# haoheliu/voicefixer

Measured on AMD Instinct MI355X. Metric: seconds-of-44.1kHz-audio restored per wall-second, higher is better.
Workload: dtype f32

## Files before the change

include/vfx_hip.h:

```cpp
#ifndef VFX_HIP_H
#define VFX_HIP_H

#include <stddef.h>
#include <stdint.h>

#ifdef __cplusplus
extern "C" {
#endif

typedef void* vfx_stream_t;

#define VFX_OK 0
#define VFX_EINVAL (-1)
#define VFX_EALIGN (-2)
#define VFX_ERANGE (-3)
#define VFX_ENOTSUP (-4)

typedef struct {
    void* ptr;
    int64_t bstride, cstride, lstride;
    int64_t guard;
    const int32_t* rows;
} vfx_tensor;

// ... 25 lines not shown

#define VFX_PAD_ZERO 0
#define VFX_PAD_REFLECT 1

int vfx_version(void);

const char* vfx_build_id(void);

uint64_t vfx_launch_count(void);

int vfx_last_conv_tile(void);


int vfx_conv1d_f32(const vfx_tensor* x, const float* w_packed, const float* bias,
                   const vfx_tensor* res, const vfx_tensor* y, int B, int Cin, int Cout, int L,
                   int k, int dilation, int pad_mode, const vfx_act* act, vfx_stream_t stream);

int vfx_conv1d_f16(const vfx_tensor* x, const void* w_f16, const float* bias, const vfx_tensor* res,
                   const vfx_tensor* y, int B, int C, int L, int dilation, const vfx_act* act, int32_t* range_flag,
                   vfx_stream_t stream);

typedef struct {
    const float* w1_direct;
    const float* bias1;
    const float* w2_direct;
    const float* bias2;
    const float* w2_wino;
    const float* w2_wino4;
    const float* w1_wino4;
} vfx_resblock_w;
int vfx_resblock_f32(const vfx_tensor* x, const vfx_tensor* y, const vfx_resblock_w* w, int B, int C, int L,
                     int dilation, float slope, int post_act, float post_slope, vfx_stream_t stream);

int vfx_convtr1d_f32(const vfx_tensor* x, const float* w_packed, const float* bias,
                     const vfx_tensor* y, int B, int Cin, int Cout, int Lin, int stride,
                     const vfx_act* act, vfx_stream_t stream);

int vfx_conv2d_f32(const vfx_tensor* x, const float* w_packed, const float* bias,
                   const vfx_tensor* res, const vfx_tensor* y, int B, int Cin, int Cout, int H,
                   int pitch_log2, int ksize, const vfx_act* act, vfx_stream_t stream);

int vfx_convtr2d_3x3s2_f32(const vfx_tensor* x, const float* w_packed, const vfx_tensor* y,
                           int B, int Cin, int Cout, int h, int in_pitch_log2,
                           const vfx_act* act, vfx_stream_t stream);

int vfx_conv1d_cout1_f32(const vfx_tensor* x, const float* w, const float* bias,
                         const vfx_tensor* y, int B, int Cin, int L, int k, int pad_mode,
                         int post_act, int out_mask_log2, vfx_stream_t stream);

int vfx_avgpool2x2_f32(const vfx_tensor* x, const vfx_tensor* y, int B, int C, int H,
                       int pitch_log2, vfx_stream_t stream);


int vfx_frontend_init(const float* window, const float* twiddle, const int32_t* lo,
                      const int32_t* hi, const int32_t* off, const float* coef, int nnz);

int vfx_frontend_readback(int which, int32_t* lo, int32_t* hi, int32_t* off, float* coef, int coef_capacity,
                          int* nnz_out);

int vfx_stft_mel_f32(const float* wav, int64_t wav_stride, int B, int N, float* mel,
                     vfx_stream_t stream);

int vfx_stft_mel_rows_f32(const float* wav, int64_t wav_stride, int B, const int32_t* n_rows, int T, float* mel,
                          vfx_stream_t stream);

int vfx_frontend_init_oracle(const int32_t* lo, const int32_t* hi, const int32_t* off, const float* coef,
// ... 48 lines not shown
```

voicefixer_amd/_lib.py:

```python
import ctypes as C
import os
import subprocess

from ._dev import dev_env

_HERE = os.path.dirname(os.path.abspath(__file__))
LIB_PATH = dev_env("VFX_LIB", os.path.join(_HERE, "libvfx_hip.so"))
CSRC = os.path.join(_HERE, "csrc")


class VfxError(RuntimeError):
    pass


class vfx_tensor(C.Structure):
    _fields_ = [("ptr", C.c_void_p), ("bstride", C.c_int64), ("cstride", C.c_int64),
                ("lstride", C.c_int64), ("guard", C.c_int64), ("rows", C.c_void_p)]


class vfx_act(C.Structure):
    _fields_ = [("pre_act", C.c_int), ("pre_slope", C.c_float), ("pre_scale", C.c_void_p),
                ("pre_shift", C.c_void_p), ("post_act", C.c_int), ("post_slope", C.c_float),
                ("math", C.c_int), ("w_x3", C.c_void_p), ("w_direct", C.c_void_p), ("w_wino4", C.c_void_p)]


class vfx_resblock_w(C.Structure):
    _fields_ = [("w1_direct", C.c_void_p), ("bias1", C.c_void_p), ("w2_direct", C.c_void_p), ("bias2", C.c_void_p),
                ("w2_wino", C.c_void_p), ("w2_wino4", C.c_void_p), ("w1_wino4", C.c_void_p)]


PRE_NONE, PRE_LRELU, PRE_AFFINE_LRELU = 0, 1, 2
POST_NONE, POST_LRELU, POST_ELU, POST_TANH, POST_SIGMOID, POST_LRELU_SNAKE = 0, 1, 2, 3, 4, 5
PAD_ZERO, PAD_REFLECT = 0, 1
MATH_F32, MATH_BF16X3 = 0, 1
EINVAL, EALIGN, ERANGE, ENOTSUP = -1, -2, -3, -4

_T = C.POINTER(vfx_tensor)
_A = C.POINTER(vfx_act)
_P = C.c_void_p
_I = C.c_int

SIGNATURES = {
    "vfx_version": (_I, []),
    "vfx_build_id": (C.c_char_p, []),
    "vfx_launch_count": (C.c_uint64, []),
    "vfx_last_conv_tile": (_I, []),
    "vfx_conv1d_f32": (_I, [_T, _P, _P, _T, _T, _I, _I, _I, _I, _I, _I, _I, _A, _P]),
    "vfx_conv1d_f16": (_I, [_T, _P, _P, _T, _T, _I, _I, _I, _I, _A, _P, _P]),
    "vfx_resblock_f32": (_I, [_T, _T, C.POINTER(vfx_resblock_w), _I, _I, _I, _I, C.c_float, _I, C.c_float, _P]),
    "vfx_convtr1d_f32": (_I, [_T, _P, _P, _T, _I, _I, _I, _I, _I, _A, _P]),
    "vfx_conv2d_f32": (_I, [_T, _P, _P, _T, _T, _I, _I, _I, _I, _I, _I, _A, _P]),
    "vfx_convtr2d_3x3s2_f32": (_I, [_T, _P, _T, _I, _I, _I, _I, _I, _A, _P]),
    "vfx_conv1d_cout1_f32": (_I, [_T, _P, _P, _T, _I, _I, _I, _I, _I, _I, _I, _P]),
    "vfx_avgpool2x2_f32": (_I, [_T, _T, _I, _I, _I, _I, _P]),
    "vfx_frontend_init": (_I, [_P, _P, _P, _P, _P, _P, _I]),
    "vfx_frontend_readback": (_I, [_I, _P, _P, _P, _P, _I, C.POINTER(_I)]),
    "vfx_stft_mel_f32": (_I, [_P, C.c_int64, _I, _I, _P, _P]),
    "vfx_stft_mel_rows_f32": (_I, [_P, C.c_int64, _I, _P, _I, _P, _P]),
    "vfx_post_rows_f32": (_I, [_P, C.c_int64, _I, _P, _P, C.c_int64, _P, _I, _I, _P, _P]),
    "vfx_mel_to_cond_rows_f32": (_I, [_P, _T, _I, _I, _P, _I, _P]),
    "vfx_frontend_init_oracle": (_I, [_P, _P, _P, _P, _I]),
    "vfx_peak_f32": (_I, [_P, C.c_int64, _I, _I, _P, _P]),
    "vfx_stft_mel_oracle_f32": (_I, [_P, C.c_int64, _I, _I, _P, _P, _P]),
    "vfx_mel_to_cond_ex_f32": (_I, [_P, _T, _I, _I, _I, _P]),
    "vfx_hf_workspace_bytes": (C.c_size_t, [_I, _I]),
    "vfx_hf_cut_f32": (_I, [_P, C.c_int64, _I, _I, _P, C.c_int64, C.c_float, _P, C.c_size_t, _P, _P]),
    "vfx_tm_to_cm_f32": (_I, [_P, _P, _I, _I, _I, C.c_int64, C.c_int64, _P]),
    "vfx_unet_input_f32": (_I, [_P, _T, _T, _I, _I, _I, _I, _P]),
    "vfx_unet_output_f32": (_I, [_T, _T, _P, _T, _P, _P, _I, _I, _I, _P]),
    "vfx_gru_bidir_f32": (_I, [_P, _P, _P, _T, _I, _I, _P]),
    "vfx_gru_bidir2_f32": (_I, [_P, _P, _P, _T, _I, _I, _P, C.c_size_t, _P, _P]),
    "vfx_gru_layout": (None, [C.POINTER(_I), C.POINTER(_I), C.POINTER(_I)]),
    "vfx_mel_to_cond_f32": (_I, [_P, _T, _I, _I, _P]),
    "vfx_post_f32": (_I, [_P, C.c_int64, _I, _P, C.c_int64, _I, _I, _P, _P]),
}

_lib = None


def build(verbose=False):
    r = subprocess.run(["make", "-C", CSRC, "-j8"], capture_output=True, text=True)
    if verbose or r.returncode != 0:
# ... 28 lines not shown
```

voicefixer_amd/csrc/vfx_conv.hip:

```cpp
#include "vfx_common.h"
#include <cstdio>
#include <cstdlib>
#include <cstring>
#include <map>
#include <mutex>
#include <string>
#include <type_traits>
#include <vector>

#ifndef VFX_X3_ABL
#define VFX_X3_ABL 0
#endif
#ifndef VFX_ABL
#define VFX_ABL 0
#endif
#define VFX_MAXPH 8
#define VFX_MAXT 9

typedef float f32x16 __attribute__((ext_vector_type(16)));
typedef unsigned int u32x4 __attribute__((ext_vector_type(4)));

#if VFX_ABL & 8
__device__ unsigned long long g_dbg[10];
__device__ unsigned long long g_dbgx[6];
// ... 53 lines not shown
    int q_shift, q_mask, o_rs, o_cs;
    int pad_mode, pre_act, post_act;
    float pre_slope, post_slope;
    int in_mask, out_mask;
    int tile_lo, tile_hi;
    int tpw;
    int x_guard;
    int ksplit, cpp, ws_ls;
    float* ws;
    int bl_step;
    int nxv;
    int res_init;
    const void* w3;
    const ConvTables* tab3;
    int segw3;
    int xplane3;
    int buf3;
    int bl3;
    int xrow3, wrow3;
    const float* wd;
    int kcx;
    int ntiles_l, xcd_chunk;
    int nph_fold;
    int wg_d;
    const int* x_rows;
    int lq_extra;
    int stagger, stagger_wgs;
    int w_tap0, w_tapstep, w_slab0, w_slabstep, w_slab_ph, w_ooff0, w_ooff_ph, w_nseg, w_seg0, w_segstep;
    const float* wd2;
    const float* bias2;
    int yp;
    float mid_slope;
    int rb_nq1;
};

template <int KC>
struct StageCfg {
    static constexpr int MAXXV = 4;
    static constexpr int MAXWV = KC == 16 ? 6 : (KC == 8 ? 4 : 5);
};

template <int MAXXV, int MAXWV>
struct StageState {
    int x_l[MAXXV];
    int x_kc[MAXXV];
    int x_off[MAXXV];
    int w_off[MAXWV];
    float4 xv[MAXXV];
    float4 wv[MAXWV];
};

template <bool FAST, int MAXXV, int MAXWV>
__device__ __forceinline__ void stage_load(StageState<MAXXV, MAXWV>& st, const ConvArgs& a,
                                           const float* __restrict__ xb, int xcs, int c0, int lshift,
                                           __amdgpu_buffer_rsrc_t xrsrc, __amdgpu_buffer_rsrc_t wrsrc, int Lin_row) {
    if constexpr (FAST) {
        const int xso = (c0 * xcs + lshift) * 4, wso = c0 * a.Cout * 4;
#pragma unroll
        for (int j = 0; j < MAXXV; ++j) {
            const u32x4 r = __builtin_amdgcn_raw_buffer_load_b128(xrsrc, st.x_off[j], xso, 0);
            st.xv[j] = make_float4(__uint_as_float(r.x), __uint_as_float(r.y), __uint_as_float(r.z), __uint_as_float(r.w));
        }
#pragma unroll
        for (int j = 0; j < MAXWV; ++j) {
            const u32x4 r = __builtin_amdgcn_raw_buffer_load_b128(wrsrc, st.w_off[j], wso, 0);
            st.wv[j] = make_float4(__uint_as_float(r.x), __uint_as_float(r.y), __uint_as_float(r.z), __uint_as_float(r.w));
// ... 908 lines not shown
    a.xs_floats = xs;
    return VFX_OK;
}



static float* splitk_workspace(hipStream_t s, size_t bytes) {
    static std::mutex mu;
    static std::map<std::pair<int, hipStream_t>, std::pair<float*, size_t>> pool;
    int dev = 0;
    if (hipGetDevice(&dev) != hipSuccess) return nullptr;
    std::lock_guard<std::mutex> lock(mu);
    auto& e = pool[std::make_pair(dev, s)];
    if (e.second < bytes) {
        static std::vector<float*> retired;
        if (e.first) retired.push_back(e.first);
        e.first = nullptr;
        e.second = 0;
        const size_t want = bytes + bytes / 2;
        if (hipMalloc((void**)&e.first, want) != hipSuccess) { e.first = nullptr; return nullptr; }
        e.second = want;
    }
    return e.first;
}


#include "vfx_convw.inc"
#include "vfx_convwg.inc"
#include "vfx_convwg4p.inc"
#include "vfx_convwg4x.inc"
#include "vfx_convtw.inc"
#include "vfx_convwg2d.inc"
#include "vfx_resblk4.inc"
#include "vfx_convh.inc"

template <int BM, int BL, int WGM, int WGL, int NT, int MODE, int ROWS = 1>
static int launch_x3_one(const ConvArgs& a, dim3 grid, size_t lds, hipStream_t s) {
    static unsigned long long attr_set = 0;
    int attr_dev = 0;
    if (hipGetDevice(&attr_dev) != hipSuccess) attr_dev = 0;
    auto kern = conv_x3_kernel<BM, BL, WGM, WGL, NT, MODE, ROWS>;
    if (!((attr_set >> (attr_dev & 63)) & 1ull)) {
        hipError_t e = hipFuncSetAttribute(reinterpret_cast<const void*>(kern),
                                           hipFuncAttributeMaxDynamicSharedMemorySize, 160 * 1024);
        if (e != hipSuccess) return (int)e;
        attr_set |= 1ull << (attr_dev & 63);
    }
    hipLaunchKernelGGL(kern, grid, dim3(256), lds, s, a);
    VFX_LAUNCHED();
    return vfx_last_error();
}

template <int BM, int BL, int WGM, int WGL>
static int launch_x3_tile(const ConvArgs& a, int nt, int mode, int rows, dim3 grid, size_t lds, hipStream_t s) {
    if (rows == 3 && nt == 3) return launch_x3_one<BM, BL, WGM, WGL, 3, 0, 3>(a, grid, lds, s);
    if (rows == 3) return launch_x3_one<BM, BL, WGM, WGL, 1, 0, 3>(a, grid, lds, s);
#define VFX_X3(NT_)                                                                                  \
    if (nt == NT_)                                                                                   \
        return mode == 2   ? launch_x3_one<BM, BL, WGM, WGL, NT_, 2>(a, grid, lds, s)                \
               : mode == 1 ? launch_x3_one<BM, BL, WGM, WGL, NT_, 1>(a, grid, lds, s)                \
                           : launch_x3_one<BM, BL, WGM, WGL, NT_, 0>(a, grid, lds, s);
    VFX_X3(1)
    VFX_X3(2)
    VFX_X3(3)
#undef VFX_X3
    return VFX_ENOTSUP;
// ... 408 lines not shown
```

voicefixer_amd/csrc/vfx_resblk4.inc:

```
__global__ __launch_bounds__(256, 2) void resblk4_kernel(const ConvArgs a) {
    constexpr int C = 64, KC = 16, NSTEP = KC / 2, S = C / KC;
    constexpr int BQ = 64, CG = 256 / BQ, NSLOT = KC / CG;
    constexpr int PLANE = KC * BQ, BUF = 6 * PLANE;
    static_assert(NSTEP / NSLOT == 2, "two k-pair steps per staged element");
    extern __shared__ __attribute__((aligned(16))) float smem[];

    const int tid = threadIdx.x, lane = tid & 63;
    const int wave = __builtin_amdgcn_readfirstlane(tid >> 6);
    const int lo = lane & 31, hi = lane >> 5;
    const int wm = wave & 1, wq = wave >> 1;
    int bx = blockIdx.x;
    if (a.xcd_chunk > 0) {
        bx = (bx & 7) * a.xcd_chunk + (bx >> 3);
        if (bx >= a.ntiles_l) return;
    }
    const int b = blockIdx.z;
    const int d = a.wg_d;
    const float inv_d = 1.0f / (float)d;
    const int Lrow = a.x_rows ? __builtin_amdgcn_readfirstlane(a.x_rows[b]) : a.Lin;
    const int q0 = bx * a.bl_step;
    if (q0 >= Lrow) return;
    const int qend = min(Lrow, q0 + a.bl_step);
    const int y0 = q0 - 1;
    const int nq1 = a.rb_nq1;
    const int xcs = (int)a.x_cs;
    auto quad_u0 = [&](int Q) {
        const int blk = fast_div(Q, d, inv_d);
        return 4 * d * blk + (Q - blk * d);
    };

    const int sq = tid % BQ, cg = tid / BQ;
    int xvoff[6];
    {
        const int p0 = y0 + quad_u0(sq);
#pragma unroll
        for (int j = 0; j < 6; ++j) {
            const int p = p0 + (j - 1) * d;
            xvoff[j] = (sq < nq1 && p >= 0 && p < Lrow) ? (cg * xcs + p) * 4 : VFX_W_OOB;
        }
    }
    const __amdgpu_buffer_rsrc_t xrsrc = __builtin_amdgcn_make_buffer_rsrc(
        const_cast<float*>(a.x) + (long long)b * a.x_bs, (short)0, 0x7fffffff, 0x00020000);
    const float slope = a.pre_slope;
    const int wcol = (sq + 32 * (cg & 1)) & 63;
    float* const wbase = smem + cg * BQ + wcol;
    float xv[NSLOT][6];
    auto x_load_part = [&](int j, int t, int s0) {
        xv[j][t] = __uint_as_float(__builtin_amdgcn_raw_buffer_load_b32(xrsrc, xvoff[t], s0 + j * CG * xcs * 4, 0));
    };
    auto x_load = [&](int chunk) {
        const int s0 = chunk * KC * xcs * 4;
#pragma unroll
        for (int j = 0; j < NSLOT; ++j)
#pragma unroll
            for (int t = 0; t < 6; ++t) x_load_part(j, t, s0);
    };
    auto x_transform = [&](int j, float (&V)[6]) {
        float e[6];
#pragma unroll
        for (int t = 0; t < 6; ++t) e[t] = fmaxf(xv[j][t], xv[j][t] * slope);
        const float s1 = fmaf(-4.f, e[2], e[4]), s2 = fmaf(-4.f, e[1], e[3]);
        const float s3 = e[4] - e[2], s4 = e[3] - e[1];
        V[0] = fmaf(4.f, e[0], fmaf(-5.f, e[2], e[4]));
        V[1] = s1 + s2;
        V[2] = s1 - s2;
        V[3] = fmaf(2.f, s4, s3);
        V[4] = fmaf(-2.f, s4, s3);
        V[5] = fmaf(4.f, e[1], fmaf(-5.f, e[3], e[5]));
    };
    const __amdgpu_buffer_rsrc_t wrsrc =
        __builtin_amdgcn_make_buffer_rsrc(const_cast<float*>(a.wd), (short)0, 0x7fffffff, 0x00020000);
// ... 76 lines not shown
        x_load(1);
        __builtin_amdgcn_sched_barrier(0);
    }
    __syncthreads();
    mma_chunk(std::true_type{}, smem, wbase + BUF, 2, 0);
    __syncthreads();
    mma_chunk(std::false_type{}, smem + BUF, wbase, 3, 2);
    __syncthreads();
#pragma unroll 1
    for (int s = 2; s < S; s += 2) {
        mma_chunk(std::false_type{}, smem, wbase + BUF, min(s + 2, S - 1), 2 * s);
        __syncthreads();
        mma_chunk(std::false_type{}, smem + BUF, wbase, min(s + 3, S - 1), 2 * s + 2);
        __syncthreads();
    }

    const int row2 = 32 * wm;
    const __amdgpu_buffer_rsrc_t w2rsrc =
        __builtin_amdgcn_make_buffer_rsrc(const_cast<float*>(a.wd2), (short)0, 0x7fffffff, 0x00020000);
    const __amdgpu_buffer_rsrc_t rrsrc = __builtin_amdgcn_make_buffer_rsrc(
        const_cast<float*>(a.x) + (long long)b * a.x_bs, (short)0, 0x7fffffff, 0x00020000);
    const __amdgpu_buffer_rsrc_t yrsrc = __builtin_amdgcn_make_buffer_rsrc(
        a.y + (long long)b * a.y_bs, (short)0, 0x7fffffff, 0x00020000);
    float4 aw2[2][6];
    auto a2_load = [&](auto set_tag, int grp) {
        constexpr int SET = decltype(set_tag)::value;
#pragma unroll
        for (int k = 0; k < 6; ++k) {
            const u32x4 r = __builtin_amdgcn_raw_buffer_load_b128(w2rsrc, avoff, k * pstride + grp * gstride, 0);
            aw2[SET][k] = make_float4(__uint_as_float(r.x), __uint_as_float(r.y), __uint_as_float(r.z), __uint_as_float(r.w));
        }
    };
    const int Qi = 32 * wq + lo;
    const int qq = q0 + 4 * Qi;
    const bool full = qq + 3 < qend;
    const bool has_tail = (qend & 3) != 0;
    const int rvq = full ? (4 * hi * xcs + qq) * 4 : VFX_W_OOB;
    const int yvq = full ? (4 * hi * (int)a.y_cs + qq) * 4 : VFX_W_OOB;
    int rv1[4], yv1[4];
#pragma unroll
    for (int i = 0; i < 4; ++i) {
        const bool one = !full && qq + i < qend;
        rv1[i] = one ? (4 * hi * xcs + qq + i) * 4 : VFX_W_OOB;
        yv1[i] = one ? (4 * hi * (int)a.y_cs + qq + i) * 4 : VFX_W_OOB;
    }
    u32x4 rq[16];
    {
        const int cs4 = xcs * 4;
#pragma unroll
        for (int r = 0; r < 16; ++r)
            rq[r] = __builtin_amdgcn_raw_buffer_load_b128(rrsrc, rvq, (row2 + (r & 3) + 8 * (r >> 2)) * cs4, 0);
    }
    a2_load(S0{}, 0);
    u32x4 bq2[4];
    {
        const __amdgpu_buffer_rsrc_t b2rsrc = __builtin_amdgcn_make_buffer_rsrc(
            const_cast<float*>(a.bias2 ? a.bias2 : a.x), (short)0, 0x7fffffff, 0x00020000);
        const int bvoff = a.bias2 ? (row2 + 4 * hi) * 4 : VFX_W_OOB;
#pragma unroll
        for (int g = 0; g < 4; ++g) bq2[g] = __builtin_amdgcn_raw_buffer_load_b128(b2rsrc, bvoff, g * 32, 0);
    }
    float* const Y = smem;
    const int yp = a.yp;
    {
        const float ms = a.mid_slope;
        const int Q1 = 32 * wq + lo;
        const int u0 = quad_u0(Q1);
        bool ok[4];
#pragma unroll
        for (int i = 0; i < 4; ++i) {
            const int p = y0 + u0 + i * d;
            ok[i] = p >= 0 && p < Lrow;
        }
        if (Q1 < nq1) {
            float* ycol = Y + (row1 + 4 * hi) * yp + u0;
#pragma unroll
            for (int r = 0; r < 16; ++r) {
                const float p12 = acc[1][r] + acc[2][r], m12 = acc[1][r] - acc[2][r];
                const float p34 = acc[3][r] + acc[4][r], m34 = acc[3][r] - acc[4][r];
                float v[4];
                v[0] = (acc[0][r] + p12) + p34;
                v[1] = fmaf(2.f, m34, m12);
                v[2] = fmaf(4.f, p34, p12);
                v[3] = fmaf(8.f, m34, m12) + acc[5][r];
                float* yr = ycol + ((r & 3) + 8 * (r >> 2)) * yp;
#pragma unroll
                for (int i = 0; i < 4; ++i) yr[i * d] = ok[i] ? fmaxf(v[i], v[i] * ms) : 0.f;
            }
        }
    }
    __syncthreads();

    f32x16 accq[6];
#pragma unroll
    for (int r = 0; r < 16; ++r) {
        accq[0][r] = __uint_as_float(rq[r].x); accq[1][r] = __uint_as_float(rq[r].y);
        accq[3][r] = __uint_as_float(rq[r].z); accq[5][r] = __uint_as_float(rq[r].w);
    }
    if (has_tail) {
        const int cs4 = xcs * 4;
#pragma unroll
        for (int r = 0; r < 16; ++r) {
            const int soff = (row2 + (r & 3) + 8 * (r >> 2)) * cs4;
            accq[0][r] += __uint_as_float(__builtin_amdgcn_raw_buffer_load_b32(rrsrc, rv1[0], soff, 0));
            accq[1][r] += __uint_as_float(__builtin_amdgcn_raw_buffer_load_b32(rrsrc, rv1[1], soff, 0));
            accq[3][r] += __uint_as_float(__builtin_amdgcn_raw_buffer_load_b32(rrsrc, rv1[2], soff, 0));
            accq[5][r] += __uint_as_float(__builtin_amdgcn_raw_buffer_load_b32(rrsrc, rv1[3], soff, 0));
        }
    }
#pragma unroll
    for (int g = 0; g < 4; ++g) {
#pragma unroll
        for (int e = 0; e < 4; ++e) {
            const int r = 4 * g + e;
            const float bb = __uint_as_float(e == 0 ? bq2[g].x : (e == 1 ? bq2[g].y : (e == 2 ? bq2[g].z : bq2[g].w)));
            const float t0 = accq[0][r] + bb, t1 = accq[1][r] + bb, t2 = accq[3][r] + bb, t3 = accq[5][r] + bb;
            const float m3 = 0.5f * (t2 - t1);
            const float m1 = 2.f * t1 - t2;
            accq[0][r] = t0 - m1 - m3;
            accq[1][r] = m1;
            accq[2][r] = 0.f;
            accq[3][r] = m3;
            accq[4][r] = 0.f;
            accq[5][r] = t3 - m1 - 8.f * m3;
        }
    }
    const float* yb = Y + hi * yp + 4 * Qi;
    auto group = [&](auto set_tag, int grp, int nxt) {
        constexpr int SET = decltype(set_tag)::value;
        const float* yg = yb + grp * 8 * yp;
        float4 dl = *reinterpret_cast<const float4*>(yg);
        float2 dh = *reinterpret_cast<const float2*>(yg + 4);
#pragma unroll
        for (int kk = 0; kk < 4; ++kk) {
            float V[6];
            {
                const float s1 = fmaf(-4.f, dl.z, dh.x), s2 = fmaf(-4.f, dl.y, dl.w);
                const float s3 = dh.x - dl.z, s4 = dl.w - dl.y;
                V[0] = fmaf(4.f, dl.x, fmaf(-5.f, dl.z, dh.x));
                V[1] = s1 + s2;
                V[2] = s1 - s2;
                V[3] = fmaf(2.f, s4, s3);
                V[4] = fmaf(-2.f, s4, s3);
                V[5] = fmaf(4.f, dl.y, fmaf(-5.f, dl.w, dh.y));
            }
            if (kk < 3) {
                dl = *reinterpret_cast<const float4*>(yg + (kk + 1) * 2 * yp);
                dh = *reinterpret_cast<const float2*>(yg + (kk + 1) * 2 * yp + 4);
            }
            if (kk == 0) {
                if constexpr (SET == 0) a2_load(S1{}, nxt);
                else a2_load(S0{}, nxt);
            }
            __builtin_amdgcn_sched_barrier(0);
#pragma unroll
            for (int k = 0; k < 6; ++k) {
                const float4 av4 = aw2[SET][k];
                const float av = kk == 0 ? av4.x : (kk == 1 ? av4.y : (kk == 2 ? av4.z : av4.w));
                accq[k] = __builtin_amdgcn_mfma_f32_32x32x2f32(av, V[k], accq[k], 0, 0, 0);
            }
// ... 25 lines not shown
#pragma unroll
                for (int i = 0; i < 4; ++i) __builtin_amdgcn_raw_buffer_store_b32(__float_as_uint(v[i]), yrsrc, yv1[i], soff, 0);
            }
        };
        if (post == VFX_POST_NONE) {
#pragma unroll
            for (int r = 0; r < 16; ++r) {
                float y[4];
                outs(r, y);
                store4(y, (row2 + (r & 3) + 8 * (r >> 2)) * cs4);
            }
        } else if (post == VFX_POST_LRELU) {
#pragma unroll
            for (int r = 0; r < 16; ++r) {
                float y[4];
                outs(r, y);
#pragma unroll
                for (int i = 0; i < 4; ++i) y[i] = fmaxf(y[i], y[i] * ps);
                store4(y, (row2 + (r & 3) + 8 * (r >> 2)) * cs4);
            }
        } else {
#pragma unroll 1
            for (int r = 0; r < 16; ++r) {
                float y[4];
                outs(r, y);
#pragma unroll
                for (int i = 0; i < 4; ++i) y[i] = vfx_post(y[i], post, ps);
                store4(y, (row2 + (r & 3) + 8 * (r >> 2)) * cs4);
            }
        }
    }
}

extern "C" int vfx_resblock_f32(const vfx_tensor* x, const vfx_tensor* y, const vfx_resblock_w* w, int B, int C, int L,
                                int dilation, float slope, int post_act, float post_slope, vfx_stream_t stream) {
    if (!w) return VFX_EINVAL;
    const float *w1_direct = w->w1_direct, *bias1 = w->bias1, *w2_direct = w->w2_direct, *bias2 = w->bias2;
    const float *w2_wino = w->w2_wino, *w2_wino4 = w->w2_wino4, *w1_wino4 = w->w1_wino4;
    static const bool off = (VFX_DEV_ENV("VFX_FUSE_WINO44") && atoi(VFX_DEV_ENV("VFX_FUSE_WINO44")) == 0) ||
                            (VFX_DEV_ENV("VFX_FUSE_WINO4") && atoi(VFX_DEV_ENV("VFX_FUSE_WINO4")) == 0) ||
                            (VFX_DEV_ENV("VFX_FUSE_WINO") && atoi(VFX_DEV_ENV("VFX_FUSE_WINO")) == 0);
    bool ok = !off && x && y && x->ptr && y->ptr && w1_wino4 && w2_wino4 && C == 64 && B > 0 && B <= 65535 && L > 0 && dilation >= 1 &&
              dilation <= 32 && x->ptr != y->ptr;
    if (ok) {
        ok = vfx_aligned16(w1_wino4) && vfx_aligned16(w2_wino4) && vfx_aligned16(x->ptr) && vfx_aligned16(y->ptr) && x->lstride == 1 &&
             y->lstride == 1 && ((x->cstride | x->bstride | y->cstride | y->bstride) & 3) == 0 &&
             (!bias1 || vfx_aligned16(bias1)) && (!bias2 || vfx_aligned16(bias2)) && slope >= 0.f && slope <= 1.f &&
             !(post_act == VFX_POST_LRELU && !(post_slope >= 0.f && post_slope <= 1.f)) &&
             ((long long)C * x->cstride + L) * 4 < (1ll << 31) - (1ll << 20) && ((long long)C * y->cstride + L) * 4 < (1ll << 31) - (1ll << 20);
    }
    const int nb = ok ? 256 / (4 * dilation) : 0;
    if (!ok || nb < 1 || nb * dilation < 48) {
        return resblock_convw(x, y, w1_direct, bias1, w2_direct, bias2, w2_wino, w2_wino4, B, C, L, dilation, slope, post_act,
                              post_slope, stream);
    }
    ConvArgs a;
    std::memset(&a, 0, sizeof(a));
    a.x = (const float*)x->ptr;
    a.wd = w1_wino4;
    a.wd2 = w2_wino4;
    a.bias = bias1;
    a.bias2 = bias2;
    a.y = (float*)y->ptr;
    a.B = B; a.Cin = C; a.CinPad = C; a.Cout = C;
    a.Lin = L; a.Lq = L; a.Lout = L;
    a.x_bs = x->bstride; a.x_cs = x->cstride;
    a.x_rows = x->rows;
    a.y_bs = y->bstride; a.y_cs = y->cstride; a.y_ls = 1;
    a.pre_act = VFX_PRE_LRELU;
    a.pre_slope = slope;
    a.mid_slope = slope;
    a.post_act = post_act;
    a.post_slope = post_slope;
    a.wg_d = dilation;
    const int W = 4 * dilation * nb;
    const int nq2 = (W - 2) / 4;
    a.rb_nq1 = nb * dilation;
    a.bl_step = 4 * nq2;
    a.yp = 260;
    const int ntiles = (L + a.bl_step - 1) / a.bl_step;
    const size_t lds = (size_t)C * a.yp * sizeof(float);
    const dim3 grid(convw_grid_x(a, ntiles), 1, B);
    static unsigned long long attr_set = 0;
    int attr_dev = 0;
    if (hipGetDevice(&attr_dev) != hipSuccess) attr_dev = 0;
    if (!((attr_set >> (attr_dev & 63)) & 1ull)) {
        hipError_t e = hipFuncSetAttribute(reinterpret_cast<const void*>(resblk4_kernel), hipFuncAttributeMaxDynamicSharedMemorySize,
                                           160 * 1024);
        if (e != hipSuccess) return (int)e;
        attr_set |= 1ull << (attr_dev & 63);
    }
    g_last_tile = C * 100000 + 256 * 100 + 96;
    hipLaunchKernelGGL(resblk4_kernel, grid, dim3(256), lds, (hipStream_t)stream, a);
    VFX_LAUNCHED();
    return vfx_last_error();
}
```

voicefixer_amd/engine.py:

```python
import contextlib
import math

import torch

from . import ops, packing, weights
from ._lib import (PRE_NONE, PRE_LRELU, PRE_AFFINE_LRELU, POST_NONE, POST_LRELU, POST_ELU, POST_TANH,
                   POST_SIGMOID, POST_LRELU_SNAKE, PAD_ZERO, PAD_REFLECT, VfxError)


class DeviceFlagRaised(VfxError):
    gru = False
    f16 = False


class GruHandoffMissed(DeviceFlagRaised):
    """The two-CU GRU's bounded spin expired (a partner workgroup was not resident in time)."""


class F16RangeExceeded(DeviceFlagRaised):
    """An activation operand of an f16 launch (vfx_conv1d_f16) was not finite or outside the fp16 range: the call's result
    is unspecified and is re-run in fp32."""


def _up4(n):
# ... 10 lines not shown
        ops.with_rows(v, rows)
    return v


class RaggedRows:

    VOC_MULTS = (1, 7, 49, 147, 441)

    def __init__(self, lengths, device):
        n = torch.as_tensor(list(lengths), dtype=torch.int64)
        T = 1 + n // 441
        Tp = (T + 63) // 64 * 64
        Tc = T + T % 2 + 4
        table = [n, T] + [(Tp >> k) << (7 - k) for k in range(7)] + [Tc * m for m in self.VOC_MULTS]
        dev = torch.stack(table).to(torch.int32).to(device)
        self.n, self.T = dev[0], dev[1]
        self.unet = [dev[2 + k] for k in range(7)]
        self.voc = {int(m): dev[9 + i] for i, m in enumerate(self.VOC_MULTS)}
        self.T_max, self.n_max = int(T.max()), int(n.max())
        self.B = len(n)


def _dev(t, device):
    return t.contiguous().float().to(device)


def _wpair(w_packed, device):
    return _dev(w_packed, device), _dev(packing.pack_direct(w_packed), device)


from ._dev import dev_env as _dev_env
_FUSE = _dev_env("VFX_FUSE", "1") != "0"
_UNFUSE_WIDE = _dev_env("VFX_UNFUSE_WIDE", "1") != "0"
FUSE_MAX_C = 128
WINO_MIN_C = int(_dev_env("VFX_WINO_MIN_C", "128"))
WINO2D = _dev_env("VFX_WINO2D", "1") != "0"


_ARITH = {"winograd": True}


def set_winograd(on):
    _ARITH["winograd"] = bool(on)


def _wg(w):
    return w if _ARITH["winograd"] else None


MATHS = ("f32", "bf16x3", "f16")
F16_CHANNELS = (128, 256, 512)


class VocoderEngine:

    def __init__(self, state, device="cuda", math="f32"):
        sd = weights.normalise_vocoder_keys(state)
        weights.check_state(sd, weights.vocoder_manifest(), "vocoder")
        self.device = device
        self.set_math(math)

        def wn(prefix):
            return weights.fold_weight_norm(sd[prefix + ".parametrizations.weight.original0"].float(),
                                            sd[prefix + ".parametrizations.weight.original1"].float())

        self.condnet = []
# ... 95 lines not shown
        B = cond.shape[0]
        dev = cond.device
        rows = (lambda mult: ragged.voc[mult]) if ragged is not None else (lambda mult: None)
        a = _rows(B, weights.COND_CHANNELS, Tc, G_TILE, dev, rows(1))
        b = _rows(B, weights.COND_CHANNELS, Tc, G_TILE, dev, rows(1))
        x = cond
        for i, (w, wd, bias, wg) in enumerate(self.condnet):
            y = a if i % 2 == 0 else b
            ops.conv1d(x, w, bias, y, Tc, 3, 1, PAD_ZERO, self.act_elu, w3=self._x3(w), wd=wd,
                       wg4=_wg(wg) if self.math != "bf16x3" else None)
            x = y
        if stages is not None:
            stages["condnet"] = x[:, :, :Tc]
        h = _rows(B, weights.VOC_CHANNELS, Tc, G_TILE, dev, rows(1))
        ops.conv1d(x, self.pre[0], self.pre[1], h, Tc, 7, 1, PAD_REFLECT, self.act_pre)
        L = Tc
        c = weights.VOC_CHANNELS
        nst = len(self.stages)
        mult = 1
        for j, (s, upw, layers) in enumerate(self.stages):
            Lo = L * s
            c //= 2
            mult *= s
            wino = layers[0][7] is not None and c >= WINO_MIN_C and self.math != "bf16x3" and _ARITH["winograd"]
            fused = (_FUSE and self.math != "bf16x3" and c <= FUSE_MAX_C and not wino and
                     not (self.math == "f16" and c in F16_CHANNELS) and
                     c * (_up4(Lo) + 2 * (G_DIL + 4)) * 4 < 2 ** 31 - 2 ** 21)
            xs = _rows(B, c, Lo, G_DIL, dev, rows(mult))
            ys = _rows(B, c, Lo, G_DIL if fused else G_TILE, dev, rows(mult))
            ops.convtr1d(h, upw[0], upw[2], xs, L, s, self.act_none, w3=self._x3(upw[0]), wd=upw[1],
                         wg4=_wg(upw[3]) if self.math != "bf16x3" else None)
            if stages is not None:
                stages["up%d" % (j + 1)] = xs[:, :, :Lo].clone()
            first_unfused = None
            if (fused and _UNFUSE_WIDE and c == 64 and _ARITH["winograd"] and all(l[7] is not None and l[8] is not None for l in layers)
                    and B * Lo >= 1 << 18):
                wide = [i for i in range(len(layers) - 1) if 3 ** i > 27 and i % 2 == 0]
                first_unfused = wide[0] if wide else None
                assert first_unfused is None or first_unfused % 2 == 0
            for i, (w1, w1d, b1, w2, w2d, b2, w2g, w1g4, w2g4) in enumerate(layers):
                last = i == len(layers) - 1
                if fused and (first_unfused is None or i < first_unfused):
                    post, pslope = POST_NONE, 0.0
                    if last:
                        post, pslope = (POST_LRELU if j == nst - 1 else POST_LRELU_SNAKE), 0.2
                    src, dst = (xs, ys) if i % 2 == 0 else (ys, xs)
                    ops.resblock(src, dst, w1d, b1, w2d, b2, Lo, 3 ** i, 0.01, post, pslope, w2g=_wg(w2g), w2g4=_wg(w2g4),
                                 w1g4=_wg(w1g4))
                    continue
                if not wino and not fused:
                    w1g4 = w2g4 = None
                f16 = self.math == "f16" and c in F16_CHANNELS
                if not (f16 and self._conv_f16(xs, w1, b1, ys, Lo, 3 ** i, self.act_c1)):
                    ops.conv1d(xs, w1, b1, ys, Lo, 3, 3 ** i, PAD_ZERO, self.act_c1, w3=self._x3(w1), wd=w1d, wg4=_wg(w1g4))
                act = self.act_none if not last else (self.act_last if j == nst - 1 else self.act_last_snake)
                if not (f16 and self._conv_f16(ys, w2, b2, xs, Lo, 1, act, res=xs)):
                    ops.conv1d(ys, w2, b2, xs, Lo, 3, 1, PAD_ZERO, act, res=xs, w3=self._x3(w2), wd=w2d, wg4=_wg(w2g4))
            assert len(layers) % 2 == 0
            h = xs
            L = Lo
            del ys
        wav = torch.empty((B, 1, _up4(L)), device=dev)
        ops.conv1d_cout1(h, self.post[0], self.post[1], wav, L, 7, PAD_REFLECT, POST_TANH)
        return wav, L

    def forward(self, mel, T, ragged=None, stages=None):
        B = mel.shape[0]
        Tc = T + T % 2 + 4
        if ragged is None:
            cond = _rows(B, weights.N_MELS, Tc, G_TILE, mel.device)
            ops.mel_to_cond(mel, cond, T)
            if stages is not None:
                stages["cond"] = cond[:, :, :Tc].clone()
            return self.forward_cond(cond, Tc, stages=stages)
        cond = _rows(B, weights.N_MELS, Tc, G_TILE, mel.device, ragged.voc[1])
        ops.mel_to_cond(mel, cond, T, ragged.T)
        return self.forward_cond(cond, Tc, ragged=ragged)


# ... 423 lines not shown
```

voicefixer_amd/ops.py:

```python
import ctypes as C

import torch

from . import _lib
from ._lib import (vfx_tensor, vfx_act, check, PRE_NONE, PRE_LRELU, PRE_AFFINE_LRELU, POST_NONE,
                   POST_LRELU, POST_ELU, POST_TANH, POST_SIGMOID, POST_LRELU_SNAKE, PAD_ZERO,
                   PAD_REFLECT, MATH_F32, MATH_BF16X3)


def _stream():
    return C.c_void_p(torch.cuda.current_stream().cuda_stream)


def _need_cuda(*ts):
    for t in ts:
        if t is not None and not t.is_cuda:
            raise _lib.VfxError("libvfx_hip operates on device tensors only (got a CPU tensor)")


def tdesc(t):
    assert t.dim() == 3 and t.dtype == torch.float32
    rows = getattr(t, "_vfx_rows", None)
    return vfx_tensor(t.data_ptr(), t.stride(0), t.stride(1), t.stride(2), getattr(t, "_vfx_guard", 0),
                      rows.data_ptr() if rows is not None else None)
# ... 90 lines not shown
                                   C.byref(yd), B, cin, cout, L, k, dilation, pad_mode, _act(act, w3, wd, wg4), _stream())
    check(rc, "vfx_conv1d_f32")
    _prof_end(e0, B * L * cin * cout * k)


def conv1d_f16(x, w16, bias, y, L, dilation, act=None, res=None, flag=None):
    _need_cuda(x, w16, y, res, bias, flag)
    assert w16.dtype == torch.float16
    B, cn = x.shape[0], x.shape[1]
    xd, yd = tdesc(x), tdesc(y)
    rd = tdesc(res) if res is not None else None
    e0 = _prof_begin()
    rc = _lib.lib().vfx_conv1d_f16(C.byref(xd), _ptr(w16), _ptr(bias), C.byref(rd) if rd is not None else None,
                                   C.byref(yd), B, cn, L, dilation, _act(act), _ptr(flag), _stream())
    if rc == _lib.ENOTSUP:
        return False
    check(rc, "vfx_conv1d_f16")
    _prof_end(e0, B * L * cn * cn * 3)
    return True


def resblock(x, y, w1d, b1, w2d, b2, L, dilation, slope=0.01, post=POST_NONE, post_slope=0.0, w2g=None, w2g4=None, w1g4=None):
    _need_cuda(x, y, w1d, b1, w2d, b2, w2g, w2g4, w1g4)
    B, Cn = x.shape[0], x.shape[1]
    xd, yd = tdesc(x), tdesc(y)
    e0 = _prof_begin()
    wts = _lib.vfx_resblock_w(_ptr(w1d), _ptr(b1), _ptr(w2d), _ptr(b2), _ptr(w2g), _ptr(w2g4), _ptr(w1g4))
    rc = _lib.lib().vfx_resblock_f32(C.byref(xd), C.byref(yd), C.byref(wts), B, Cn, L, dilation, float(slope), post,
                                     float(post_slope), _stream())
    check(rc, "vfx_resblock_f32")
    _prof_end(e0, 2 * B * L * Cn * Cn * 3)


def convtr1d(x, w, bias, y, Lin, stride, act=None, w3=None, wd=None, wg4=None):
    _need_cuda(x, w, y, bias)
    B, cin = x.shape[0], x.shape[1]
    cout = w.shape[2]
    xd, yd = tdesc(x), tdesc(y)
    e0 = _prof_begin()
    rc = _lib.lib().vfx_convtr1d_f32(C.byref(xd), _ptr(w), _ptr(bias), C.byref(yd), B, cin, cout, Lin, stride,
                                     _act(act, w3, wd, wg4), _stream())
    check(rc, "vfx_convtr1d_f32")
    _prof_end(e0, B * Lin * cin * cout * 2 * stride)


def conv2d(x, w, bias, y, H, pitch_log2, ksize, act=None, res=None, cin=None, w3=None, wd=None, wg4=None):
    _need_cuda(x, w, y, res, bias)
    B = x.shape[0]
    cin = x.shape[1] if cin is None else cin
    cout = w.shape[2]
    xd, yd = tdesc(x), tdesc(y)
    rd = tdesc(res) if res is not None else None
    e0 = _prof_begin()
    rc = _lib.lib().vfx_conv2d_f32(C.byref(xd), _ptr(w), _ptr(bias), C.byref(rd) if rd is not None else None,
                                   C.byref(yd), B, cin, cout, H, pitch_log2, ksize, _act(act, w3, wd, wg4), _stream())
    check(rc, "vfx_conv2d_f32")
    _prof_end(e0, B * H * ((1 << pitch_log2) - 1) * cin * cout * ksize * ksize)


def convtr2d_3x3s2(x, w, y, h, in_pitch_log2, act=None, w3=None):
    _need_cuda(x, w, y)
    B, cin = x.shape[0], x.shape[1]
    cout = w.shape[2]
    xd, yd = tdesc(x), tdesc(y)
    e0 = _prof_begin()
    rc = _lib.lib().vfx_convtr2d_3x3s2_f32(C.byref(xd), _ptr(w), C.byref(yd), B, cin, cout, h, in_pitch_log2,
# ... 178 lines not shown
```

Measured before the change: 1580.

## Add strip-tiled fused Winograd-4 resblock kernel for large dilations at 64 channels

Templates the fused Winograd F(4,3) resblock kernel body on a STRIP mode. The new mode tiles the sequence in strips of 32 or 64 positions, each strip holding a residue class of the dilation. That lets dilations too large for the original tile scheme (past 27 at 64 channels) still run both convolutions of the residual block in one kernel instead of falling back to the unfused path. The engine routes a whole 64-channel stage through this entry point by default, which also bypasses the existing unfuse-wide heuristic. The trade-off is more halo recomputation and more index arithmetic per strip at large dilations.

```diff
diff --git a/include/vfx_hip.h b/include/vfx_hip.h
--- a/include/vfx_hip.h
+++ b/include/vfx_hip.h
@@ -81,6 +81,9 @@
 int vfx_resblock_f32(const vfx_tensor* x, const vfx_tensor* y, const vfx_resblock_w* w, int B, int C, int L,
                      int dilation, float slope, int post_act, float post_slope, vfx_stream_t stream);
 
+int vfx_resblock_wino4_f32(const vfx_tensor* x, const vfx_tensor* y, const vfx_resblock_w* w, int B, int C, int L,
+                           int dilation, float slope, int post_act, float post_slope, vfx_stream_t stream);
+
 int vfx_convtr1d_f32(const vfx_tensor* x, const float* w_packed, const float* bias,
                      const vfx_tensor* y, int B, int Cin, int Cout, int Lin, int stride,
                      const vfx_act* act, vfx_stream_t stream);
diff --git a/voicefixer_amd/_lib.py b/voicefixer_amd/_lib.py
--- a/voicefixer_amd/_lib.py
+++ b/voicefixer_amd/_lib.py
@@ -48,6 +48,7 @@
     "vfx_conv1d_f32": (_I, [_T, _P, _P, _T, _T, _I, _I, _I, _I, _I, _I, _I, _A, _P]),
     "vfx_conv1d_f16": (_I, [_T, _P, _P, _T, _T, _I, _I, _I, _I, _A, _P, _P]),
     "vfx_resblock_f32": (_I, [_T, _T, C.POINTER(vfx_resblock_w), _I, _I, _I, _I, C.c_float, _I, C.c_float, _P]),
+    "vfx_resblock_wino4_f32": (_I, [_T, _T, C.POINTER(vfx_resblock_w), _I, _I, _I, _I, C.c_float, _I, C.c_float, _P]),
     "vfx_convtr1d_f32": (_I, [_T, _P, _P, _T, _I, _I, _I, _I, _I, _A, _P]),
     "vfx_conv2d_f32": (_I, [_T, _P, _P, _T, _T, _I, _I, _I, _I, _I, _I, _A, _P]),
     "vfx_convtr2d_3x3s2_f32": (_I, [_T, _P, _T, _I, _I, _I, _I, _I, _A, _P]),
diff --git a/voicefixer_amd/csrc/vfx_conv.hip b/voicefixer_amd/csrc/vfx_conv.hip
--- a/voicefixer_amd/csrc/vfx_conv.hip
+++ b/voicefixer_amd/csrc/vfx_conv.hip
@@ -109,6 +109,7 @@
     int yp;
     float mid_slope;
     int rb_nq1;
+    int rs_pshift, rs_nseg;
 };
 
 template <int KC>
@@ -1083,6 +1084,7 @@
 #include "vfx_convtw.inc"
 #include "vfx_convwg2d.inc"
 #include "vfx_resblk4.inc"
+#include "vfx_resblk4s.inc"
 #include "vfx_convh.inc"
 
 template <int BM, int BL, int WGM, int WGL, int NT, int MODE, int ROWS = 1>
diff --git a/voicefixer_amd/csrc/vfx_resblk4.inc b/voicefixer_amd/csrc/vfx_resblk4.inc
--- a/voicefixer_amd/csrc/vfx_resblk4.inc
+++ b/voicefixer_amd/csrc/vfx_resblk4.inc
@@ -1,4 +1,5 @@
-__global__ __launch_bounds__(256, 2) void resblk4_kernel(const ConvArgs a) {
+template <bool STRIP>
+__device__ __forceinline__ void resblk4_body(const ConvArgs& a) {
     constexpr int C = 64, KC = 16, NSTEP = KC / 2, S = C / KC;
     constexpr int BQ = 64, CG = 256 / BQ, NSLOT = KC / CG;
     constexpr int PLANE = KC * BQ, BUF = 6 * PLANE;
@@ -18,25 +19,50 @@
     const int d = a.wg_d;
     const float inv_d = 1.0f / (float)d;
     const int Lrow = a.x_rows ? __builtin_amdgcn_readfirstlane(a.x_rows[b]) : a.Lin;
-    const int q0 = bx * a.bl_step;
-    if (q0 >= Lrow) return;
-    const int qend = min(Lrow, q0 + a.bl_step);
-    const int y0 = q0 - 1;
+    const int xcs = (int)a.x_cs;
+    const int q0 = STRIP ? 0 : bx * a.bl_step;
     const int nq1 = a.rb_nq1;
-    const int xcs = (int)a.x_cs;
+    const int pshift = STRIP ? a.rs_pshift : 6, P = 1 << pshift, W = P - 4;
+    int sstart[2] = {0, 0}, sr0[2] = {0, 0};
+    if constexpr (STRIP) {
+        const int nseg = a.rs_nseg;
+        const float inv_nseg = 1.0f / (float)nseg;
+#pragma unroll
+        for (int g = 0; g < 2; ++g) {
+            const int n = (bx << (6 - pshift)) + g;
+            const int blk = fast_div(n, nseg, inv_nseg);
+            sr0[g] = (n - blk * nseg) * W;
+            sstart[g] = 4 * d * blk + sr0[g];
+        }
+    }
+    if ((STRIP ? sstart[0] : q0) >= Lrow) return;
     auto quad_u0 = [&](int Q) {
         const int blk = fast_div(Q, d, inv_d);
         return 4 * d * blk + (Q - blk * d);
     };
+    auto quad_p = [&](int Q) {
+        if constexpr (STRIP) return (Q >> pshift ? sstart[1] : sstart[0]) - 1 + (Q & (P - 1));
+        else return q0 - 1 + quad_u0(Q);
+    };
+    auto quad_ok = [&](int Q) {
+        if constexpr (STRIP) return (Q & (P - 1)) < P - 2;
+        else return Q < nq1;
+    };
+    auto quad_col = [&](int Q) {
+        if constexpr (STRIP) return ((Q >> pshift) << (pshift + 2)) + (Q & (P - 1));
+        else return quad_u0(Q);
+    };
+    const int ystep = STRIP ? P : d;
 
     const int sq = tid % BQ, cg = tid / BQ;
     int xvoff[6];
     {
-        const int p0 = y0 + quad_u0(sq);
+        const int p0 = quad_p(sq);
+        const bool qok = quad_ok(sq);
 #pragma unroll
         for (int j = 0; j < 6; ++j) {
             const int p = p0 + (j - 1) * d;
-            xvoff[j] = (sq < nq1 && p >= 0 && p < Lrow) ? (cg * xcs + p) * 4 : VFX_W_OOB;
+            xvoff[j] = (qok && p >= 0 && p < Lrow) ? (cg * xcs + p) * 4 : VFX_W_OOB;
         }
     }
     const __amdgpu_buffer_rsrc_t xrsrc = __builtin_amdgcn_make_buffer_rsrc(
@@ -179,15 +205,33 @@
         }
     };
     const int Qi = 32 * wq + lo;
-    const int qq = q0 + 4 * Qi;
-    const bool full = qq + 3 < qend;
-    const bool has_tail = (qend & 3) != 0;
+    int qq, nown, yc2;
+    bool has_tail;
+    if constexpr (STRIP) {
+        const int nq2s = W >> 2;
+        int t = fast_div(Qi, nq2s, 1.0f / (float)nq2s);
+        const int jq = Qi - t * nq2s;
+        const bool sok = t < (4 << (6 - pshift));
+        t = sok ? t : 0;
+        const int rr = ((t >> 2) ? sr0[1] : sr0[0]) + 4 * jq;
+        qq = ((t >> 2) ? sstart[1] : sstart[0]) + (t & 3) * d + 4 * jq;
+        nown = sok ? min(Lrow - qq, d - rr) : 0;
+        has_tail = __any(nown > 0 && nown < 4);
+        yc2 = (t << pshift) + 4 * jq;
+    } else {
+        const int qend = min(Lrow, q0 + a.bl_step);
+        qq = q0 + 4 * Qi;
+        nown = qend - qq;
+        has_tail = (qend & 3) != 0;
+        yc2 = 4 * Qi;
+    }
+    const bool full = nown >= 4;
     const int rvq = full ? (4 * hi * xcs + qq) * 4 : VFX_W_OOB;
     const int yvq = full ? (4 * hi * (int)a.y_cs + qq) * 4 : VFX_W_OOB;
     int rv1[4], yv1[4];
 #pragma unroll
     for (int i = 0; i < 4; ++i) {
-        const bool one = !full && qq + i < qend;
+        const bool one = !full && i < nown;
         rv1[i] = one ? (4 * hi * xcs + qq + i) * 4 : VFX_W_OOB;
         yv1[i] = one ? (4 * hi * (int)a.y_cs + qq + i) * 4 : VFX_W_OOB;
     }
@@ -212,15 +256,15 @@
     {
         const float ms = a.mid_slope;
         const int Q1 = 32 * wq + lo;
-        const int u0 = quad_u0(Q1);
+        const int p1 = quad_p(Q1);
         bool ok[4];
 #pragma unroll
         for (int i = 0; i < 4; ++i) {
-            const int p = y0 + u0 + i * d;
+            const int p = p1 + i * d;
             ok[i] = p >= 0 && p < Lrow;
         }
-        if (Q1 < nq1) {
-            float* ycol = Y + (row1 + 4 * hi) * yp + u0;
+        if (quad_ok(Q1)) {
+            float* ycol = Y + (row1 + 4 * hi) * yp + quad_col(Q1);
 #pragma unroll
             for (int r = 0; r < 16; ++r) {
                 const float p12 = acc[1][r] + acc[2][r], m12 = acc[1][r] - acc[2][r];
@@ -232,7 +276,7 @@
                 v[3] = fmaf(8.f, m34, m12) + acc[5][r];
                 float* yr = ycol + ((r & 3) + 8 * (r >> 2)) * yp;
 #pragma unroll
-                for (int i = 0; i < 4; ++i) yr[i * d] = ok[i] ? fmaxf(v[i], v[i] * ms) : 0.f;
+                for (int i = 0; i < 4; ++i) yr[i * ystep] = ok[i] ? fmaxf(v[i], v[i] * ms) : 0.f;
             }
         }
     }
@@ -272,7 +316,7 @@
             accq[5][r] = t3 - m1 - 8.f * m3;
         }
     }
-    const float* yb = Y + hi * yp + 4 * Qi;
+    const float* yb = Y + hi * yp + yc2;
     auto group = [&](auto set_tag, int grp, int nxt) {
         constexpr int SET = decltype(set_tag)::value;
         const float* yg = yb + grp * 8 * yp;
@@ -364,16 +408,14 @@
     }
 }
 
-extern "C" int vfx_resblock_f32(const vfx_tensor* x, const vfx_tensor* y, const vfx_resblock_w* w, int B, int C, int L,
-                                int dilation, float slope, int post_act, float post_slope, vfx_stream_t stream) {
-    if (!w) return VFX_EINVAL;
-    const float *w1_direct = w->w1_direct, *bias1 = w->bias1, *w2_direct = w->w2_direct, *bias2 = w->bias2;
-    const float *w2_wino = w->w2_wino, *w2_wino4 = w->w2_wino4, *w1_wino4 = w->w1_wino4;
-    static const bool off = (VFX_DEV_ENV("VFX_FUSE_WINO44") && atoi(VFX_DEV_ENV("VFX_FUSE_WINO44")) == 0) ||
-                            (VFX_DEV_ENV("VFX_FUSE_WINO4") && atoi(VFX_DEV_ENV("VFX_FUSE_WINO4")) == 0) ||
-                            (VFX_DEV_ENV("VFX_FUSE_WINO") && atoi(VFX_DEV_ENV("VFX_FUSE_WINO")) == 0);
-    bool ok = !off && x && y && x->ptr && y->ptr && w1_wino4 && w2_wino4 && C == 64 && B > 0 && B <= 65535 && L > 0 && dilation >= 1 &&
-              dilation <= 32 && x->ptr != y->ptr;
+__global__ __launch_bounds__(256, 2) void resblk4_kernel(const ConvArgs a) { resblk4_body<false>(a); }
+
+
+static bool resblk4_args_ok(const vfx_tensor* x, const vfx_tensor* y, const vfx_resblock_w* w, int B, int C, int L, int dilation,
+                            float slope, int post_act, float post_slope) {
+    const float *bias1 = w->bias1, *bias2 = w->bias2, *w2_wino4 = w->w2_wino4, *w1_wino4 = w->w1_wino4;
+    bool ok = x && y && x->ptr && y->ptr && w1_wino4 && w2_wino4 && C == 64 && B > 0 && B <= 65535 && L > 0 && dilation >= 1 &&
+              x->ptr != y->ptr;
     if (ok) {
         ok = vfx_aligned16(w1_wino4) && vfx_aligned16(w2_wino4) && vfx_aligned16(x->ptr) && vfx_aligned16(y->ptr) && x->lstride == 1 &&
              y->lstride == 1 && ((x->cstride | x->bstride | y->cstride | y->bstride) & 3) == 0 &&
@@ -381,18 +423,17 @@
              !(post_act == VFX_POST_LRELU && !(post_slope >= 0.f && post_slope <= 1.f)) &&
              ((long long)C * x->cstride + L) * 4 < (1ll << 31) - (1ll << 20) && ((long long)C * y->cstride + L) * 4 < (1ll << 31) - (1ll << 20);
     }
-    const int nb = ok ? 256 / (4 * dilation) : 0;
-    if (!ok || nb < 1 || nb * dilation < 48) {
-        return resblock_convw(x, y, w1_direct, bias1, w2_direct, bias2, w2_wino, w2_wino4, B, C, L, dilation, slope, post_act,
-                              post_slope, stream);
-    }
-    ConvArgs a;
+    return ok;
+}
+
+static void resblk4_fill_args(ConvArgs& a, const vfx_tensor* x, const vfx_tensor* y, const vfx_resblock_w* w, int B, int C, int L,
+                              int dilation, float slope, int post_act, float post_slope) {
     std::memset(&a, 0, sizeof(a));
     a.x = (const float*)x->ptr;
-    a.wd = w1_wino4;
-    a.wd2 = w2_wino4;
-    a.bias = bias1;
-    a.bias2 = bias2;
+    a.wd = w->w1_wino4;
+    a.wd2 = w->w2_wino4;
+    a.bias = w->bias1;
+    a.bias2 = w->bias2;
     a.y = (float*)y->ptr;
     a.B = B; a.Cin = C; a.CinPad = C; a.Cout = C;
     a.Lin = L; a.Lq = L; a.Lout = L;
@@ -405,11 +446,23 @@
     a.post_act = post_act;
     a.post_slope = post_slope;
     a.wg_d = dilation;
+    a.yp = 260;
+}
+
+static bool resblk4_takes(int dilation) {
+    const int nb = 256 / (4 * dilation);
+    return dilation <= 32 && nb >= 1 && nb * dilation >= 48;
+}
+
+static int resblk4_launch(const vfx_tensor* x, const vfx_tensor* y, const vfx_resblock_w* w, int B, int C, int L, int dilation,
+                          float slope, int post_act, float post_slope, vfx_stream_t stream) {
+    ConvArgs a;
+    resblk4_fill_args(a, x, y, w, B, C, L, dilation, slope, post_act, post_slope);
+    const int nb = 256 / (4 * dilation);
     const int W = 4 * dilation * nb;
     const int nq2 = (W - 2) / 4;
     a.rb_nq1 = nb * dilation;
     a.bl_step = 4 * nq2;
-    a.yp = 260;
     const int ntiles = (L + a.bl_step - 1) / a.bl_step;
     const size_t lds = (size_t)C * a.yp * sizeof(float);
     const dim3 grid(convw_grid_x(a, ntiles), 1, B);
@@ -427,3 +480,16 @@
     VFX_LAUNCHED();
     return vfx_last_error();
 }
+
+extern "C" int vfx_resblock_f32(const vfx_tensor* x, const vfx_tensor* y, const vfx_resblock_w* w, int B, int C, int L,
+                                int dilation, float slope, int post_act, float post_slope, vfx_stream_t stream) {
+    if (!w) return VFX_EINVAL;
+    static const bool off = (VFX_DEV_ENV("VFX_FUSE_WINO44") && atoi(VFX_DEV_ENV("VFX_FUSE_WINO44")) == 0) ||
+                            (VFX_DEV_ENV("VFX_FUSE_WINO4") && atoi(VFX_DEV_ENV("VFX_FUSE_WINO4")) == 0) ||
+                            (VFX_DEV_ENV("VFX_FUSE_WINO") && atoi(VFX_DEV_ENV("VFX_FUSE_WINO")) == 0);
+    if (off || !resblk4_takes(dilation) || !resblk4_args_ok(x, y, w, B, C, L, dilation, slope, post_act, post_slope)) {
+        return resblock_convw(x, y, w->w1_direct, w->bias1, w->w2_direct, w->bias2, w->w2_wino, w->w2_wino4, B, C, L, dilation, slope,
+                              post_act, post_slope, stream);
+    }
+    return resblk4_launch(x, y, w, B, C, L, dilation, slope, post_act, post_slope, stream);
+}
diff --git a/voicefixer_amd/csrc/vfx_resblk4s.inc b/voicefixer_amd/csrc/vfx_resblk4s.inc
--- /dev/null
+++ b/voicefixer_amd/csrc/vfx_resblk4s.inc
@@ -0,0 +1,35 @@
+__global__ __launch_bounds__(256, 2) void resblk4s_kernel(const ConvArgs a) { resblk4_body<true>(a); }
+
+extern "C" int vfx_resblock_wino4_f32(const vfx_tensor* x, const vfx_tensor* y, const vfx_resblock_w* w, int B, int C, int L,
+                                      int dilation, float slope, int post_act, float post_slope, vfx_stream_t stream) {
+    if (!w) return VFX_EINVAL;
+    if (!resblk4_args_ok(x, y, w, B, C, L, dilation, slope, post_act, post_slope)) return VFX_ENOTSUP;
+    if (resblk4_takes(dilation)) return resblk4_launch(x, y, w, B, C, L, dilation, slope, post_act, post_slope, stream);
+    ConvArgs a;
+    resblk4_fill_args(a, x, y, w, B, C, L, dilation, slope, post_act, post_slope);
+    auto nseg_of = [&](int P) { return (dilation + P - 5) / (P - 4); };
+    const int pshift = 32 * nseg_of(32) < 64 * nseg_of(64) ? 5 : 6;
+    const int nseg = nseg_of(1 << pshift);
+    a.rs_pshift = pshift;
+    a.rs_nseg = nseg;
+    const long long nblk = ((long long)L + 4ll * dilation - 1) / (4ll * dilation);
+    const long long nsegs = nblk * nseg;
+    const int G = 64 >> pshift;
+    const long long ntiles = (nsegs + G - 1) / G;
+    if (ntiles * G >= (1 << 20)) return VFX_ENOTSUP;
+    const size_t lds = (size_t)C * a.yp * sizeof(float);
+    const dim3 grid(convw_grid_x(a, (int)ntiles), 1, B);
+    static unsigned long long attr_set = 0;
+    int attr_dev = 0;
+    if (hipGetDevice(&attr_dev) != hipSuccess) attr_dev = 0;
+    if (!((attr_set >> (attr_dev & 63)) & 1ull)) {
+        hipError_t e = hipFuncSetAttribute(reinterpret_cast<const void*>(resblk4s_kernel), hipFuncAttributeMaxDynamicSharedMemorySize,
+                                           160 * 1024);
+        if (e != hipSuccess) return (int)e;
+        attr_set |= 1ull << (attr_dev & 63);
+    }
+    g_last_tile = C * 100000 + 256 * 100 + 97;
+    hipLaunchKernelGGL(resblk4s_kernel, grid, dim3(256), lds, (hipStream_t)stream, a);
+    VFX_LAUNCHED();
+    return vfx_last_error();
+}
diff --git a/voicefixer_amd/engine.py b/voicefixer_amd/engine.py
--- a/voicefixer_amd/engine.py
+++ b/voicefixer_amd/engine.py
@@ -66,6 +66,7 @@
 from ._dev import dev_env as _dev_env
 _FUSE = _dev_env("VFX_FUSE", "1") != "0"
 _UNFUSE_WIDE = _dev_env("VFX_UNFUSE_WIDE", "1") != "0"
+_WINO4_STAGE = _dev_env("VFX_WINO4_STAGE", "1") != "0"
 FUSE_MAX_C = 128
 WINO_MIN_C = int(_dev_env("VFX_WINO_MIN_C", "128"))
 WINO2D = _dev_env("VFX_WINO2D", "1") != "0"
@@ -227,8 +228,10 @@
                          wg4=_wg(upw[3]) if self.math != "bf16x3" else None)
             if stages is not None:
                 stages["up%d" % (j + 1)] = xs[:, :, :Lo].clone()
+            wino4_stage = (fused and _WINO4_STAGE and c == 64 and _ARITH["winograd"] and
+                           all(l[7] is not None and l[8] is not None for l in layers))
             first_unfused = None
-            if (fused and _UNFUSE_WIDE and c == 64 and _ARITH["winograd"] and all(l[7] is not None and l[8] is not None for l in layers)
+            if (fused and not wino4_stage and _UNFUSE_WIDE and c == 64 and _ARITH["winograd"] and all(l[7] is not None and l[8] is not None for l in layers)
                     and B * Lo >= 1 << 18):
                 wide = [i for i in range(len(layers) - 1) if 3 ** i > 27 and i % 2 == 0]
                 first_unfused = wide[0] if wide else None
@@ -240,6 +243,9 @@
                     if last:
                         post, pslope = (POST_LRELU if j == nst - 1 else POST_LRELU_SNAKE), 0.2
                     src, dst = (xs, ys) if i % 2 == 0 else (ys, xs)
+                    if wino4_stage:
+                        ops.resblock_wino4(src, dst, _wg(w1g4), b1, _wg(w2g4), b2, Lo, 3 ** i, 0.01, post, pslope)
+                        continue
                     ops.resblock(src, dst, w1d, b1, w2d, b2, Lo, 3 ** i, 0.01, post, pslope, w2g=_wg(w2g), w2g4=_wg(w2g4),
                                  w1g4=_wg(w1g4))
                     continue
diff --git a/voicefixer_amd/ops.py b/voicefixer_amd/ops.py
--- a/voicefixer_amd/ops.py
+++ b/voicefixer_amd/ops.py
@@ -146,6 +146,18 @@
     _prof_end(e0, 2 * B * L * Cn * Cn * 3)
 
 
+def resblock_wino4(x, y, w1g4, b1, w2g4, b2, L, dilation, slope=0.01, post=POST_NONE, post_slope=0.0):
+    _need_cuda(x, y, w1g4, b1, w2g4, b2)
+    B, Cn = x.shape[0], x.shape[1]
+    xd, yd = tdesc(x), tdesc(y)
+    e0 = _prof_begin()
+    wts = _lib.vfx_resblock_w(None, _ptr(b1), None, _ptr(b2), None, _ptr(w2g4), _ptr(w1g4))
+    rc = _lib.lib().vfx_resblock_wino4_f32(C.byref(xd), C.byref(yd), C.byref(wts), B, Cn, L, dilation, float(slope), post,
+                                           float(post_slope), _stream())
+    check(rc, "vfx_resblock_wino4_f32")
+    _prof_end(e0, 2 * B * L * Cn * Cn * 3)
+
+
 def convtr1d(x, w, bias, y, Lin, stride, act=None, w3=None, wd=None, wg4=None):
     _need_cuda(x, w, y, bias)
     B, cin = x.shape[0], x.shape[1]
```

After: 1606 (median of 6 runs). 1.02x the previous value.
